# vita-epfl/CrowdNav

Hardware: AMD Instinct MI355X
Metric: env-steps/sec (whole node), 4096 envs x 5 humans, ORCA step (higher is better)
Workload: dtype f32 ORCA solve + f64 env step

## Files before the change

crowdnav_amd/csrc/rollout_fused.h:

```cpp
#pragma once
#include "rollout_kernels.h"

namespace cn {

constexpr int kFusedMaxNC = 5;

template <typename T>
__device__ __forceinline__ T in_vgpr(T x) {
    asm volatile("" : "+v"(x));
    return x;
}

__device__ __forceinline__ void stage_agent(const Params& P, const Smem& s, const Lane& L, const AgentRegs& r,
                                            double human_safety) {
    if (L.lane >= P.nA) return;
    s.kin[L.lane] = make_float4((float)r.px, (float)r.py, (float)r.vx, (float)r.vy);
    s.posd[L.lane] = make_double2(r.px, r.py);
    s.rad[L.lane] = r.rad;
    s.hview[L.lane] = (float)(r.rad + 0.01 + human_safety);
}

__device__ __forceinline__ void preferred_velocity(const AgentRegs& r, float max_speed, bool solve, float4& sol, float4& start) {
    const double gdx = r.gx - r.px, gdy = r.gy - r.py;
    const double speed = norm2(gdx, gdy);
    const float pref_x = (float)(speed > 1.0 ? gdx / speed : gdx);
    const float pref_y = (float)(speed > 1.0 ? gdy / speed : gdy);
    sol = make_float4(pref_x, pref_y, max_speed, solve ? 1.0f : 0.0f);
    float sx, sy;
    lp_start_point(max_speed, pref_x, pref_y, sx, sy);
    start = make_float4(sx, sy, 0.0f, 0.0f);
}

#define CN_FUSED_SYNC() wave_lds_sync()



struct PairRow {
    int my_info, my_slot;
    unsigned long long row_slots;
};
__device__ __forceinline__ PairRow pair_row_of(const Params& P, const Smem& s, int lane) {
    PairRow pr{0, P.nA, 0ull};
    if (lane < P.pairs) {
        pr.my_info = s.pinfo[lane];
        const int c = (pr.my_info >> 16) & 0xff;
        for (int k = 0; k < kFusedMaxNC; ++k) {
            int slot = P.nA;
            if (k < P.NC) {
                const int ik = s.pinfo[lane - c + k];
                slot = ((ik >> 24) & 1) ? ((ik >> 8) & 0xff) : P.nA;
            }
            pr.row_slots |= (unsigned long long)slot << (8 * k);
        }
        pr.my_slot = (int)((pr.row_slots >> (8 * c)) & 0xffull);
    }
    return pr;
}

template <typename Mid>
__device__ __forceinline__ void fused_pair_phase(const Params& P, const Smem& s, const PairRow& pr, float range_sq, Mid&& mid) {
    const int my_info = pr.my_info, my_slot = pr.my_slot;
    const unsigned long long row_slots = pr.row_slots;
    const int q = my_info & 0xff, c = (my_info >> 16) & 0xff;
    const int ol = (my_info >> 8) & 0xff;
    const bool robot_sim = (my_info >> 25) & 1;
    const float4 me = s.kin[q];
    const float4 other = s.kin[my_slot];
    float4 ot[kFusedMaxNC];
#pragma unroll
    for (int k = 0; k < kFusedMaxNC; ++k) ot[k] = s.kin[(int)((row_slots >> (8 * k)) & 0xffull)];
    const float* view = robot_sim ? s.rview : s.hview;
    const float rsum = view[q] + view[ol];
    const float odx = me.x - other.x, ody = me.y - other.y;
    const float mine = odx * odx + ody * ody;
    int rank = 0, within = 0;
    {
        const uint32_t mb = __float_as_uint(mine), rb = __float_as_uint(range_sq);
        uint32_t before = 0u, inside = 0u;
#pragma unroll
        for (int k = 0; k < kFusedMaxNC; ++k) {
            const float dx = me.x - ot[k].x, dy = me.y - ot[k].y;
            const uint32_t vb = __float_as_uint(dx * dx + dy * dy);
            const uint32_t tie = (uint32_t)(k - c) >> 31;
            before = __builtin_amdgcn_alignbit(before, vb - mb - tie, 31);
            inside = __builtin_amdgcn_alignbit(inside, vb - rb, 31);
        }
        within = __popc(inside);
        rank = __popc(before & inside);
    }
    mid();
    if (c == 0) s.count[q] = within < P.orca.max_neighbors ? within : P.orca.max_neighbors;
    if (mine < range_sq && rank < P.orca.max_neighbors)
        s.lines[q * kLineStride + rank] =
            make_half_plane(P.orca, me.x, me.y, me.z, me.w, other.x, other.y, other.z, other.w, rsum);
}

template <int MAXL>
__device__ __forceinline__ void fused_candidates(const Params& P, const Smem& s, int lane) {
    if (lane < P.nA * MAXL) {
        const int q = lane / MAXL, k = lane - q * MAXL;
        const float4 so = s.sol[q];
        const float4* lq = s.lines + q * kLineStride;
        s.cand2[q * kLineStride + k] = lp_line_candidate_pairs5(lq, k, lane, so.z, so.x, so.y);
    }
}

__device__ __forceinline__ void split_barrier() {
    asm volatile("s_waitcnt lgkmcnt(0)\n\ts_barrier" ::: "memory");
}

struct Lp3Item {
    int a, m, i, base;
    bool item;
    float4 li, lj;
    float radius;
};
template <int MAXL>
__device__ __forceinline__ Lp3Item lp3_item_of(const Smem& s, int lane, unsigned long long mask) {
    constexpr int kPairs = MAXL * (MAXL - 1) / 2;
    Lp3Item it;
    const int t = lane / kPairs;
    it.m = lane - t * kPairs;
    it.a = 0;
    unsigned long long rest = mask;
#pragma unroll
    for (int u = 0; u < kWave / kPairs; ++u) {
        const int bit = rest ? __ffsll((long long)rest) - 1 : 0;
        it.a = (u == t) ? bit : it.a;
        rest &= rest - 1ull;
    }
    it.item = lane < (int)__popcll(mask) * kPairs;
    it.i = lp3_program_of(it.m), it.base = it.i * (it.i - 1) / 2;
    const float4* la = s.lines + it.a * kLineStride;
    it.li = la[it.i], it.lj = la[it.m - it.base];
    it.radius = s.sol[it.a].z;
    return it;
}
template <int MAXL>
__device__ __forceinline__ void lp3_head(const Smem& s, const Lp3Item& it) {
    const float4 pr = lp3_project(it.li, it.lj);
    if (it.item) s.proj[it.a * kLineStride + it.m] = pr;
    CN_FUSED_SYNC();
    if (it.item) {
        const float4* pa = s.proj + it.a * kLineStride + it.base;
        s.cand3[it.a * kLineStride + it.m] =
            lp_line_candidate<MAXL - 2>(pa[it.m - it.base], pa, it.m - it.base, it.radius, -it.li.w, it.li.z, true);
    }
}

template <int MAXL>
__device__ __forceinline__ bool split_has_head(unsigned int pred, int u, int n_steps) {
    return pred != 0u && __popc(pred) * (MAXL * (MAXL - 1) / 2) <= kWave && u < n_steps;
}

struct NoOp {
    __device__ __forceinline__ void operator()() const {}
};
template <int MAXL, int BASE_PRIO = 0, typename AfterScan = NoOp>
__device__ __forceinline__ unsigned long long fused_solve(const Params& P, const Smem& s, int lane, bool solve, float& rx,
                                                          float& ry, PhaseClock* clk, unsigned long long have = 0ull,
                                                          AfterScan&& after_scan = NoOp{}) {
    (void)P, (void)clk;
    rx = 0.0f, ry = 0.0f;
    int n = 0, fail = 0;
    if (solve) {
        n = s.count[lane];
        const float4 start = s.res[lane];
        rx = start.x, ry = start.y;
        fail = lp_planar_scan<MAXL>(s.lines + lane * kLineStride, s.cand2 + lane * kLineStride, n, rx, ry);
    }
    CN_TICK(clk, 3);
    const bool need = solve && fail < n;
    const unsigned long long nm = __ballot(need);
#ifdef CN_PHASE_TIMING
    if (clk) clk->acc[9] += __popcll(nm);
#endif
    after_scan();
    if (nm == 0ull) __builtin_amdgcn_s_setprio(BASE_PRIO);
    if (nm != 0ull) {
        __builtin_amdgcn_s_setprio(3);
        constexpr int kPairs = MAXL * (MAXL - 1) / 2;
        const int n_todo = __popcll(nm);
        bool one_pass_done = false;
        if (n_todo * kPairs <= kWave) {
            const Lp3Item it = lp3_item_of<MAXL>(s, lane, nm);
            const bool item = it.item;
            const int a = it.a, i = it.i, m = it.m, base = it.base;
            const float4 li = it.li;
            const float radius = it.radius;
            const bool hit = (nm & ~have) == 0ull;
            if (!hit) {
                lp3_head<MAXL>(s, it);
                CN_FUSED_SYNC();
            }
            if (item && m == base)
                s.cand2[a * kLineStride + i] = lp3_inner_program(s.proj + a * kLineStride, s.cand3 + a * kLineStride, i, li, radius);
            CN_FUSED_SYNC();
            if (need)
                lp3_outer_scan(s.lines + lane * kLineStride, s.cand2 + lane * kLineStride, n, fail, s.sol[lane].z, rx, ry);
            one_pass_done = true;
        } else {
            if (need) s.todo[__popcll(nm & ((1ull << lane) - 1ull))] = lane;
            CN_FUSED_SYNC();
            const int items = n_todo * kPairs;
            for (int p = lane; p < items; p += kWave) {
                const int t = p / kPairs, m = p - t * kPairs;
                const int a = s.todo[t];
                const int i = lp3_program_of(m), j = m - i * (i - 1) / 2;
                const float4* la = s.lines + a * kLineStride;
                s.proj[a * kLineStride + m] = lp3_project(la[i], la[j]);
            }
            CN_FUSED_SYNC();
            for (int p = lane; p < items; p += kWave) {
                const int t = p / kPairs, m = p - t * kPairs;
                const int a = s.todo[t];
                const int i = lp3_program_of(m), base = i * (i - 1) / 2;
                const float4 li = s.lines[a * kLineStride + i];
                const float4* pa = s.proj + a * kLineStride + base;
                s.cand3[a * kLineStride + m] = lp_line_candidate<MAXL - 2>(pa[m - base], pa, m - base, s.sol[a].z, -li.w, li.z, true);
            }
            CN_FUSED_SYNC();
        }
        if (need && !one_pass_done)
            lp3_scan(s.lines + lane * kLineStride, s.proj + lane * kLineStride, s.cand3 + lane * kLineStride, n,
                     fail, s.sol[lane].z, rx, ry);
    }
    return nm;
}

struct StepConsts {
    double dt, limit, limit1, success, collision, ddist, dfactor, hsafety;
};
__device__ __forceinline__ StepConsts step_consts(const Params& P) {
    StepConsts K;
    K.dt = in_vgpr(P.dt), K.limit = in_vgpr(P.time_limit), K.limit1 = in_vgpr(P.time_limit - 1.0);
    K.success = in_vgpr(P.success_reward), K.collision = in_vgpr(P.collision_penalty);
    K.ddist = in_vgpr(P.discomfort_dist), K.dfactor = in_vgpr(P.discomfort_factor);
    K.hsafety = in_vgpr(P.human_safety);
    return K;
}

__device__ __forceinline__ double swept_distance(const AgentRegs& r, bool human, double2 rp, double act_x, double act_y,
                                                 double new_vx, double new_vy, double dt, double robot_rad) {
    const double x1 = r.px - rp.x, y1 = r.py - rp.y;
    const double wx = r.vx - act_x, wy = r.vy - act_y;
    const double x2 = x1 + wx * dt, y2 = y1 + wy * dt;
    const double sx = x2 - x1, sy = y2 - y1;
    double u = ((0.0 - x1) * sx + (0.0 - y1) * sy) / (sx * sx + sy * sy);
    u = (u > 1.0) ? 1.0 : ((u < 0.0) ? 0.0 : u);
    const bool degenerate = (sx == 0.0 && sy == 0.0);
    const double cx = degenerate ? 0.0 - x1 : (x1 + u * sx) - 0.0;
    const double cy = degenerate ? 0.0 - y1 : (y1 + u * sy) - 0.0;
    const double endx = r.px + new_vx * dt, endy = r.py + new_vy * dt;
    const double d = norm2(human ? cx : endx - r.gx, human ? cy : endy - r.gy);
    return human ? d - r.rad - robot_rad : d;
}

struct StepOutcome {
    double reward, dmin;
    int info;
    bool done;
};
__device__ __forceinline__ StepOutcome reduce_env(const Params& P, const Smem& s, int ebase, double gtime, const StepConsts& K) {
    const double goal_dist = s.closest[ebase];
    const double robot_rad = s.rad[ebase];
    double dmin = std::numeric_limits<double>::infinity();
    bool collision = false;
    for (int i = 1; i < P.A; ++i) {
        const double c = s.closest[ebase + i];
        const bool hit = c < 0.0;
        dmin = (!collision & !hit & (c < dmin)) ? c : dmin;
        collision = collision | hit;
    }
    const bool timeout = gtime >= K.limit1;
    const bool reaching = goal_dist < robot_rad;
    const bool danger = dmin < K.ddist;
    double reward = danger ? (dmin - K.ddist) * K.dfactor * K.dt : 0.0;
    int info = danger ? CN_DANGER : CN_NOTHING;
    reward = reaching ? K.success : reward, info = reaching ? CN_REACH_GOAL : info;
    reward = collision ? K.collision : reward, info = collision ? CN_COLLISION : info;
    reward = timeout ? 0.0 : reward, info = timeout ? CN_TIMEOUT : info;
    const bool done = timeout | collision | reaching;
    return StepOutcome{reward, dmin, info, done};
}


#ifdef CN_WAVE_TRACE
static __device__ unsigned long long cn_wave_trace[8192 * 6];
#endif

constexpr int kSplitOrcaPrio = 1;
constexpr int kAssistHead = 1;
#ifndef CN_SPLIT_HEAD_PRIO
#define CN_SPLIT_HEAD_PRIO 2
#endif
#ifndef CN_SPLIT_HEAD_TAIL_PRIO
#define CN_SPLIT_HEAD_TAIL_PRIO 1
#endif

#ifdef CN_SPLIT_PROBE
constexpr bool kSplitProbe = true;
static __device__ unsigned long long cn_split_probe[32];
#define SPLIT_PROBE_DECL()                                                                                   \
    unsigned long long sp_cnt[7] = {}, sp_wait[3] = {}, sp_w1[2] = {}, sp_n1[2] = {}, sp_dt = 0ull; \
    bool sp_prev_head = false
#define SPLIT_PROBE_WAIT(k, barrier)                                   \
    do {                                                               \
        const unsigned long long sp_t0 = __builtin_readcyclecounter(); \
        barrier;                                                       \
        sp_dt = __builtin_readcyclecounter() - sp_t0;                  \
        sp_wait[k] += sp_dt;                                           \
    } while (0)
#define SPLIT_PROBE_AFTER_1(word, head)                               \
    do {                                                               \
        if ((word) != 0u) sp_w1[0] += sp_dt, ++sp_n1[0];               \
        if (sp_prev_head) sp_w1[1] += sp_dt, ++sp_n1[1];               \
        sp_prev_head = (head);                                         \
    } while (0)
#define SPLIT_PROBE_STEP(ended, nm, head, pred)                                  \
    do {                                                                         \
        const bool sp_hit = (head) && (nm) != 0ull && ((nm) & ~(unsigned long long)(pred)) == 0ull; \
        ++sp_cnt[0], sp_cnt[1] += (ended) ? 1 : 0, sp_cnt[2] += (nm) != 0ull ? 1 : 0, sp_cnt[3] += (head) ? 1 : 0; \
        sp_cnt[4] += sp_hit ? 1 : 0, sp_cnt[5] += ((nm) != 0ull && !sp_hit) ? 1 : 0, sp_cnt[6] += ((head) && (nm) == 0ull) ? 1 : 0; \
    } while (0)
#define SPLIT_PROBE_FLUSH(lane, base)                                                        \
    do {                                                                                     \
        if ((lane) == 0) {                                                                   \
            if ((base) == 0)                                                                 \
                for (int k = 0; k < 7; ++k) atomicAdd(&cn_split_probe[k], sp_cnt[k]);        \
            for (int k = 0; k < 3; ++k) atomicAdd(&cn_split_probe[((base) ? 10 : 7) + k], sp_wait[k]); \
            for (int k = 0; k < 2; ++k) {                                                    \
                atomicAdd(&cn_split_probe[((base) ? 17 : 13) + k], sp_w1[k]);                \
                atomicAdd(&cn_split_probe[((base) ? 19 : 15) + k], sp_n1[k]);                \
            }                                                                                \
        }                                                                                    \
    } while (0)
#else
constexpr bool kSplitProbe = false;
#define SPLIT_PROBE_DECL() (void)0
#define SPLIT_PROBE_WAIT(k, barrier) barrier
#define SPLIT_PROBE_AFTER_1(word, head) (void)0
#define SPLIT_PROBE_STEP(ended, nm, head, pred) (void)0
#define SPLIT_PROBE_FLUSH(lane, base) (void)0
#endif

template <int MAXL, int ASSIST>
__device__ __forceinline__ void split_orca_wave(const Params& P, const Smem& s, int n_steps) {
    const int lane = (int)threadIdx.x - kWave;
    float2* const vel = reinterpret_cast<float2*>(s.act);
    const float range_sq = P.orca.neighbor_dist * P.orca.neighbor_dist;
    const double c_dt = in_vgpr(P.dt);
    split_barrier();
    __builtin_amdgcn_s_setprio(kSplitOrcaPrio);
    const PairRow pr = pair_row_of(P, s, lane);
    double px = 0.0, py = 0.0;
    float rx = 0.0f, ry = 0.0f;
    bool solved = false;
    SPLIT_PROBE_DECL();
    for (int u = 0;;) {
        SPLIT_PROBE_WAIT(0, split_barrier());
        const bool ended = __builtin_amdgcn_readfirstlane(s.flag[0]) != 0;
        const unsigned int pred = ((ASSIST & kAssistHead) || kSplitProbe) ? (unsigned int)__builtin_amdgcn_readfirstlane(s.flag[1]) : 0u;
        if (!ended) ++u;
        if (u >= n_steps) {
            split_barrier();
            break;
        }
        const bool head = (ASSIST & kAssistHead) ? split_has_head<MAXL>(pred, u, n_steps) : false;
        SPLIT_PROBE_AFTER_1(pred, head);
        if (lane < P.nA) {
            if (ended) {
                const double2 p = s.posd[lane];
                px = p.x, py = p.y;
            } else if (solved) {
                px = px + (double)rx * c_dt;
                py = py + (double)ry * c_dt;
                s.kin[lane] = make_float4((float)px, (float)py, rx, ry);
            }
        }
        CN_FUSED_SYNC();
        if (lane < P.pairs) fused_pair_phase(P, s, pr, range_sq, [] {});
        SPLIT_PROBE_WAIT(1, split_barrier());
        fused_candidates<MAXL>(P, s, lane);
        CN_FUSED_SYNC();
        solved = lane < P.nA && s.sol[lane < P.nA ? lane : 0].w != 0.0f;
        const unsigned long long nm = fused_solve<MAXL, kSplitOrcaPrio>(P, s, lane, solved, rx, ry, nullptr, head ? pred : 0u, [&] {
            if (head) SPLIT_PROBE_WAIT(2, split_barrier());
        });
        if (lane < P.nA) vel[lane] = make_float2(rx, ry);
        if (((ASSIST & kAssistHead) || kSplitProbe) && lane == 0) s.flag[1] = (int)nm;
        SPLIT_PROBE_STEP(ended, nm, head, pred);
    }
    SPLIT_PROBE_FLUSH(lane, 0);
}

template <bool HEADLINE, bool SPLIT = false, int ASSIST = 0>
__global__ __launch_bounds__((SPLIT ? 2 : 1) * kWave, (SPLIT ? 4 : HEADLINE ? 3 : 1)) void rollout_fused_kernel(
    Params P_in, const StateView* Sd, const int* ring_filled_in, RolloutView R, int n_steps, const double* ext_action) {
    static_assert(HEADLINE || !SPLIT, "the two-wave kernel exists for the headline geometry only");
    static_assert(SPLIT || ASSIST == 0, "the env wave assists an ORCA wave: two-wave kernel only");
#ifdef CN_WAVE_TRACE
    const unsigned long long wt_entry = __builtin_amdgcn_s_memrealtime();
    unsigned long long wt_fallbacks = 0ull, wt_ends = 0ull;
#endif
    constexpr int MAXL = 5;
    Params P = P_in;
    P.async_fill = 0;
    if (HEADLINE) {
        P.A = 6, P.NC = 5, P.E = 2, P.nA = 12, P.pairs = 60, P.threads = 64;
    }
    const Smem s = carve<MAXL>(P);
    if constexpr (SPLIT) {
        if (__builtin_amdgcn_readfirstlane((int)threadIdx.x) >= kWave) {
            split_orca_wave<MAXL, ASSIST>(P, s, n_steps);
            return;
        }
    }
    const Lane L = lane_of(P);
    AgentRegs r = {};
    float robot_max_speed = 0.0f;
    const bool robot = L.valid && L.a == 0;
    const cn_rollout_io* iop = R.io;
    double theta = 0.0;
    EpisodeBook ep = {};
    {
        const StateView S = *Sd;
        const cn_rollout_io io = *iop;
        const size_t gi = L.valid ? L.gi : 0;
        const int env = L.valid ? L.env : 0;
        const double2 p0 = S.pos[gi], v0 = S.vel[gi], g0 = S.goal[gi], q0 = S.rv[gi];
        const bool have = P.robot_orca ? S.rsim_valid[env] != 0 : false;
        const float rr_kept = P.robot_orca ? S.rsim_radius[gi] : 0.0f;
        const float ms_kept = P.robot_orca ? S.rsim_max_speed[env] : 0.0f;
        const double theta0 = S.theta[env];
        EpisodeBook ep0;
        CN_LOAD_EPISODE(P, ep0, S, io, ring_filled_in, env);
        if (L.valid) {
            r.px = p0.x, r.py = p0.y, r.vx = v0.x, r.vy = v0.y, r.gx = g0.x, r.gy = g0.y, r.rad = q0.x, r.vpref = q0.y;
            ep = ep0;
            if (L.a == 0) theta = theta0;
            if (P.robot_orca) {
                const float rr = have ? rr_kept : (float)(r.rad + 0.01 + P.robot_safety);
                if (!have) S.rsim_radius[L.gi] = rr;
                s.rview[L.lane] = rr;
                if (L.a == 0) {
                    robot_max_speed = have ? ms_kept : (float)r.vpref;
                    if (!have) S.rsim_max_speed[L.env] = robot_max_speed;
                }
            }
        }
    }
    build_pairs(P, s);

    if (L.valid && ep.state == kWaitingScenario && scenario_ready(P, *Sd, L.env, ep.ep_count, ep.ring_filled)) {
        load_from_ring(P, *Sd, L, ep.ep_count % P.ring_mod, r);
        ep.state = kRunning;
        ep.gtime = 0.0;
        theta = 1.5707963267948966;
    }
    unsigned int transitions = 0;
    for (int t = threadIdx.x; t < kMaxDiscount; t += P.threads) s.disc[t] = t < R.discount_len ? R.discount[t] : 0.0;
    CN_FUSED_SYNC();
    if (L.lane == 0) s.kin[P.nA] = make_float4(std::numeric_limits<float>::infinity(), std::numeric_limits<float>::infinity(), 0.0f, 0.0f);
    const PairRow pr = pair_row_of(P, s, L.lane);
    const StepConsts K = step_consts(P);
    stage_agent(P, s, L, r, K.hsafety);
    CN_FUSED_SYNC();

#ifdef CN_PHASE_TIMING
    PhaseClock clock = {};
    PhaseClock* clk = &clock;
    clock.last = __builtin_readcyclecounter();
#else
    PhaseClock* clk = nullptr;
    (void)clk;
#endif
    const float range_sq = P.orca.neighbor_dist * P.orca.neighbor_dist;
#ifdef CN_WAVE_TRACE
    const unsigned long long wt_loop = __builtin_amdgcn_s_memrealtime();
#endif
    if constexpr (SPLIT) {
        float2* const vel = reinterpret_cast<float2*>(s.act);
        if (L.lane == 0) s.flag[0] = 1, s.flag[1] = 0;
        split_barrier();
        bool skip = true;
        SPLIT_PROBE_DECL();
        for (int u = 0;;) {
            SPLIT_PROBE_WAIT(0, split_barrier());
            if (!skip) ++u;
            const unsigned int pred = ((ASSIST & kAssistHead) || kSplitProbe) ? (unsigned int)__builtin_amdgcn_readfirstlane(s.flag[1]) : 0u;
            SPLIT_PROBE_AFTER_1(pred, (ASSIST & kAssistHead) != 0 && split_has_head<MAXL>(pred, u, n_steps));
            const bool running = L.valid && ep.state == kRunning;
            const AgentRegs r0 = r;
            double act_x = 0.0, act_y = 0.0, new_vx = 0.0, new_vy = 0.0;
            if (!skip && L.lane < P.nA) {
                const float2 mine = vel[L.lane], robots = vel[L.ebase];
                act_x = (double)robots.x, act_y = (double)robots.y;
                new_vx = (L.a == 0) ? act_x : (double)mine.x;
                new_vy = (L.a == 0) ? act_y : (double)mine.y;
                if (running) {
                    r.px = r.px + new_vx * K.dt;
                    r.py = r.py + new_vy * K.dt;
                    r.vx = new_vx;
                    r.vy = new_vy;
                }
            }
            if (u < n_steps && L.lane < P.nA) {
                float4 sol4, start4;
                preferred_velocity(r, (L.a == 0) ? robot_max_speed : (float)r.vpref, running && (L.a > 0 || P.robot_orca), sol4, start4);
                s.sol[L.lane] = sol4;
                s.res[L.lane] = start4;
            }
            SPLIT_PROBE_WAIT(1, split_barrier());
            if constexpr ((ASSIST & kAssistHead) != 0) {
                if (split_has_head<MAXL>(pred, u, n_steps)) {
                    __builtin_amdgcn_s_setprio(CN_SPLIT_HEAD_PRIO);
                    const Lp3Item it = lp3_item_of<MAXL>(s, L.lane, (unsigned long long)pred);
                    lp3_head<MAXL>(s, it);
                    __builtin_amdgcn_s_setprio(CN_SPLIT_HEAD_TAIL_PRIO);
                    SPLIT_PROBE_WAIT(2, split_barrier());
                }
            }
            bool ended = false;
            if (!skip) {
                const double2 rp = make_double2(__shfl(r0.px, L.ebase), __shfl(r0.py, L.ebase));
                if (L.valid) s.closest[L.lane] = swept_distance(r0, L.a > 0, rp, act_x, act_y, new_vx, new_vy, K.dt, s.rad[L.ebase]);
                CN_FUSED_SYNC();
                bool done = false;
                if (running) {
                    const double disc_t = s.disc[ep.cur_steps < kMaxDiscount ? ep.cur_steps : kMaxDiscount - 1];
                    const StepOutcome o = reduce_env(P, s, L.ebase, ep.gtime, K);
                    done = o.done;
                    ep.gtime += K.dt;
                    ++transitions;
                    CN_BOOK_TRANSITION(ep, ep.cur_steps < kMaxDiscount ? disc_t : 0.0, o.reward, o.info, o.dmin);
                    if (done) {
                        const cn_rollout_io io = *iop;
                        const StateView S = *Sd;
                        AgentRegs next = r;
                        load_from_ring(P, S, L, (ep.ep_count + 1) % P.ring_mod, next);
                        CN_END_EPISODE(P, S, io, L.env, L.a == 0, K.limit, o.info, ep, r = next; theta = 1.5707963267948966);
                    }
                }
                ended = __ballot(done) != 0ull;
            }
            if (ended) stage_agent(P, s, L, r, K.hsafety);
            if (L.lane == 0) s.flag[0] = ended ? 1 : 0;
            skip = ended;
            if constexpr ((ASSIST & kAssistHead) != 0 && CN_SPLIT_HEAD_TAIL_PRIO != 0) __builtin_amdgcn_s_setprio(0);
            if (u >= n_steps) break;
        }
        SPLIT_PROBE_FLUSH(L.lane, 10);
    }
    const int one_wave_steps = SPLIT ? 0 : n_steps;
    for (int step = 0; step < one_wave_steps; ++step) {
        const bool running = L.valid && ep.state == kRunning;
        const bool solve = running && (L.a > 0 || P.robot_orca);

        if (L.lane < P.pairs) {
            float4 sol4, start4;
            fused_pair_phase(P, s, pr, range_sq, [&] {
                preferred_velocity(r, (L.a == 0) ? robot_max_speed : (float)r.vpref, solve, sol4, start4);
            });
            if (L.lane < P.nA) {
                s.sol[L.lane] = sol4;
                s.res[L.lane] = start4;
            }
        }
        CN_FUSED_SYNC();
        CN_TICK(clk, 2);

        fused_candidates<MAXL>(P, s, L.lane);
        CN_FUSED_SYNC();

        float rx, ry;
        const bool fell_back = fused_solve<MAXL>(P, s, L.lane, solve, rx, ry, clk) != 0ull;
        (void)fell_back;
#ifdef CN_WAVE_TRACE
        if (fell_back) ++wt_fallbacks;
#endif
        CN_TICK(clk, 8);

        double act_x, act_y;
        if (P.robot_orca) {
            act_x = (double)__shfl(rx, L.ebase);
            act_y = (double)__shfl(ry, L.ebase);
        } else {
            act_x = L.valid ? ext_action[2 * (size_t)L.env] : 0.0;
            act_y = L.valid ? ext_action[2 * (size_t)L.env + 1] : 0.0;
        }
        const double new_vx = (L.a == 0) ? act_x : (double)rx;
        const double new_vy = (L.a == 0) ? act_y : (double)ry;

        if (L.valid)
            s.closest[L.lane] = swept_distance(r, L.a > 0, s.posd[L.ebase], act_x, act_y, new_vx, new_vy, K.dt, s.rad[L.ebase]);
        CN_FUSED_SYNC();
        CN_TICK(clk, 5);

        if (running) {
            const double disc_t = s.disc[ep.cur_steps < kMaxDiscount ? ep.cur_steps : kMaxDiscount - 1];
            const StepOutcome o = reduce_env(P, s, L.ebase, ep.gtime, K);
            const double reward = o.reward, dmin = o.dmin;
            const int info = o.info;
            const bool done = o.done;
            ep.gtime += K.dt;
            r.px = r.px + new_vx * K.dt;
            r.py = r.py + new_vy * K.dt;
            r.vx = new_vx;
            r.vy = new_vy;
            ++transitions;
            CN_BOOK_TRANSITION(ep, ep.cur_steps < kMaxDiscount ? disc_t : 0.0, reward, info, dmin);
#ifdef CN_WAVE_TRACE
            if (__ballot(done) != 0ull) ++wt_ends;
#endif
            if (done) {
                const cn_rollout_io io = *iop;
                CN_END_EPISODE(P, *Sd, io, L.env, L.a == 0, K.limit, info, ep,
                               load_from_ring(P, *Sd, L, ep.ep_count % P.ring_mod, r); theta = 1.5707963267948966);
            }
        }
        stage_agent(P, s, L, r, K.hsafety);
        CN_FUSED_SYNC();
        CN_TICK(clk, 7);
    }
#ifdef CN_PHASE_TIMING
    if ((threadIdx.x & (kWave - 1)) == 0) {
        unsigned long long total = 0ull;
        for (int k = 0; k < 10; ++k) {
            atomicAdd(&cn_phase_cycles[k], clock.acc[k]);
            if (k != 9) total += clock.acc[k];
        }
        atomicMax(&cn_phase_cycles[14], total);
        atomicMin(&cn_phase_cycles[13], total);
        atomicAdd(&cn_phase_cycles[15], 1ull);
    }
#endif

#ifdef CN_WAVE_TRACE
    const unsigned long long wt_exit = __builtin_amdgcn_s_memrealtime();
#endif
    const StateView S = *Sd;
    if (L.valid) CN_STORE_AGENT(S, L.gi, r);
    const cn_rollout_io io = *iop;
    if (robot) CN_STORE_EPISODE(P, S, io, L.env, ep, theta);
    rollout_epilogue(P, S, io, L, robot, transitions, ep.ep_count, reinterpret_cast<double*>(s.lines));
#ifdef CN_WAVE_TRACE
    if (threadIdx.x == 0 && blockIdx.x < 8192) {
        unsigned long long* w = cn_wave_trace + 6 * blockIdx.x;
        unsigned hw;
        asm volatile("s_getreg_b32 %0, hwreg(HW_REG_HW_ID)" : "=s"(hw));
        w[0] = wt_entry, w[1] = wt_loop, w[2] = wt_exit, w[3] = __builtin_amdgcn_s_memrealtime();
        w[4] = wt_fallbacks | (wt_ends << 32), w[5] = hw;
    }
#endif
}

}
```

Baseline: 1.478 billion.

## Shorten the ORCA wave's step loop with bpermute distances, hoisted loads and mirrored preferred-velocity lanes

The pair phase now fetches neighbour distances from peer lanes with ds_bpermute instead of reloading five kin entries per lane and recomputing them. In the split kernel the ORCA wave does the kin position update at the end of its own step, loads me/other before the ended check, staggers episode-end staging through a separate d2 buffer, and recomputes rsum and solved only when an episode ends. This drops one LDS sync from the common path. The env wave mirrors agent state onto lanes 16+ so the x and y parts of the preferred velocity are computed in parallel and swapped with permlane16_swap. The risk is extra cross-lane state and subtle correctness dependencies, such as stale rsum or solved values, and mirror lanes that need nA <= 16.

```diff
diff --git a/crowdnav_amd/csrc/rollout_fused.h b/crowdnav_amd/csrc/rollout_fused.h
--- a/crowdnav_amd/csrc/rollout_fused.h
+++ b/crowdnav_amd/csrc/rollout_fused.h
@@ -12,9 +12,9 @@
 }
 
 __device__ __forceinline__ void stage_agent(const Params& P, const Smem& s, const Lane& L, const AgentRegs& r,
-                                            double human_safety) {
+                                            double human_safety, float4* kin) {
     if (L.lane >= P.nA) return;
-    s.kin[L.lane] = make_float4((float)r.px, (float)r.py, (float)r.vx, (float)r.vy);
+    kin[L.lane] = make_float4((float)r.px, (float)r.py, (float)r.vx, (float)r.vy);
     s.posd[L.lane] = make_double2(r.px, r.py);
     s.rad[L.lane] = r.rad;
     s.hview[L.lane] = (float)(r.rad + 0.01 + human_safety);
@@ -36,51 +36,45 @@
 
 
 struct PairRow {
-    int my_info, my_slot;
-    unsigned long long row_slots;
+    int my_info, my_slot, xbase;
 };
 __device__ __forceinline__ PairRow pair_row_of(const Params& P, const Smem& s, int lane) {
-    PairRow pr{0, P.nA, 0ull};
+    PairRow pr{0, P.nA, 0};
     if (lane < P.pairs) {
         pr.my_info = s.pinfo[lane];
         const int c = (pr.my_info >> 16) & 0xff;
-        for (int k = 0; k < kFusedMaxNC; ++k) {
-            int slot = P.nA;
-            if (k < P.NC) {
-                const int ik = s.pinfo[lane - c + k];
-                slot = ((ik >> 24) & 1) ? ((ik >> 8) & 0xff) : P.nA;
-            }
-            pr.row_slots |= (unsigned long long)slot << (8 * k);
-        }
-        pr.my_slot = (int)((pr.row_slots >> (8 * c)) & 0xffull);
+        pr.xbase = (lane - c) * 4;
+        pr.my_slot = ((pr.my_info >> 24) & 1) ? ((pr.my_info >> 8) & 0xff) : P.nA;
     }
     return pr;
 }
 
+__device__ __forceinline__ float pair_rsum(const Smem& s, const PairRow& pr) {
+    const int q = pr.my_info & 0xff, ol = (pr.my_info >> 8) & 0xff;
+    const float* view = ((pr.my_info >> 25) & 1) ? s.rview : s.hview;
+    return view[q] + view[ol];
+}
+
 template <typename Mid>
-__device__ __forceinline__ void fused_pair_phase(const Params& P, const Smem& s, const PairRow& pr, float range_sq, Mid&& mid) {
-    const int my_info = pr.my_info, my_slot = pr.my_slot;
-    const unsigned long long row_slots = pr.row_slots;
+__device__ __forceinline__ void fused_pair_body(const Params& P, const Smem& s, const PairRow& pr, float range_sq, float rsum,
+                                                const float4 me, const float4 other, Mid&& mid) {
+    const int my_info = pr.my_info;
     const int q = my_info & 0xff, c = (my_info >> 16) & 0xff;
-    const int ol = (my_info >> 8) & 0xff;
-    const bool robot_sim = (my_info >> 25) & 1;
-    const float4 me = s.kin[q];
-    const float4 other = s.kin[my_slot];
-    float4 ot[kFusedMaxNC];
-#pragma unroll
-    for (int k = 0; k < kFusedMaxNC; ++k) ot[k] = s.kin[(int)((row_slots >> (8 * k)) & 0xffull)];
-    const float* view = robot_sim ? s.rview : s.hview;
-    const float rsum = view[q] + view[ol];
     const float odx = me.x - other.x, ody = me.y - other.y;
     const float mine = odx * odx + ody * ody;
+    uint32_t vbk[kFusedMaxNC];
+#pragma unroll
+    for (int k = 0; k < kFusedMaxNC; ++k) {
+        const uint32_t got = (uint32_t)__builtin_amdgcn_ds_bpermute(pr.xbase + 4 * k, (int)__float_as_uint(mine));
+        vbk[k] = k < P.NC ? got : 0x7f800000u;
+    }
     int rank = 0, within = 0;
     {
         const uint32_t mb = __float_as_uint(mine), rb = __float_as_uint(range_sq);
         uint32_t before = 0u, inside = 0u;
 #pragma unroll
         for (int k = 0; k < kFusedMaxNC; ++k) {
-            const float dx = me.x - ot[k].x, dy = me.y - ot[k].y;
-            const uint32_t vb = __float_as_uint(dx * dx + dy * dy);
+            const uint32_t vb = vbk[k];
             const uint32_t tie = (uint32_t)(k - c) >> 31;
             before = __builtin_amdgcn_alignbit(before, vb - mb - tie, 31);
             inside = __builtin_amdgcn_alignbit(inside, vb - rb, 31);
@@ -93,6 +87,13 @@
     if (mine < range_sq && rank < P.orca.max_neighbors)
         s.lines[q * kLineStride + rank] =
             make_half_plane(P.orca, me.x, me.y, me.z, me.w, other.x, other.y, other.z, other.w, rsum);
+}
+template <typename Mid>
+__device__ __forceinline__ void fused_pair_phase(const Params& P, const Smem& s, const PairRow& pr, float range_sq, float rsum,
+                                                 Mid&& mid) {
+    const float4 me = s.kin[pr.my_info & 0xff];
+    const float4 other = s.kin[pr.my_slot];
+    fused_pair_body(P, s, pr, range_sq, rsum, me, other, mid);
 }
 
 template <int MAXL>
@@ -356,11 +357,15 @@
     double px = 0.0, py = 0.0;
     float rx = 0.0f, ry = 0.0f;
     bool solved = false;
+    float rsum = 0.0f;
+    const int pq = pr.my_info & 0xff;
     SPLIT_PROBE_DECL();
     for (int u = 0;;) {
         SPLIT_PROBE_WAIT(0, split_barrier());
-        const bool ended = __builtin_amdgcn_readfirstlane(s.flag[0]) != 0;
-        const unsigned int pred = ((ASSIST & kAssistHead) || kSplitProbe) ? (unsigned int)__builtin_amdgcn_readfirstlane(s.flag[1]) : 0u;
+        const int2 words = make_int2(s.flag[0], ((ASSIST & kAssistHead) || kSplitProbe) ? s.flag[1] : 0);
+        float4 me = s.kin[pq], other = s.kin[pr.my_slot];
+        const bool ended = __builtin_amdgcn_readfirstlane(words.x) != 0;
+        const unsigned int pred = ((ASSIST & kAssistHead) || kSplitProbe) ? (unsigned int)__builtin_amdgcn_readfirstlane(words.y) : 0u;
         if (!ended) ++u;
         if (u >= n_steps) {
             split_barrier();
@@ -368,27 +373,31 @@
         }
         const bool head = (ASSIST & kAssistHead) ? split_has_head<MAXL>(pred, u, n_steps) : false;
         SPLIT_PROBE_AFTER_1(pred, head);
-        if (lane < P.nA) {
-            if (ended) {
+        if (ended) {
+            if (lane < P.nA) {
                 const double2 p = s.posd[lane];
                 px = p.x, py = p.y;
-            } else if (solved) {
-                px = px + (double)rx * c_dt;
-                py = py + (double)ry * c_dt;
-                s.kin[lane] = make_float4((float)px, (float)py, rx, ry);
-            }
-        }
-        CN_FUSED_SYNC();
-        if (lane < P.pairs) fused_pair_phase(P, s, pr, range_sq, [] {});
+                s.kin[lane] = reinterpret_cast<const float4*>(s.d2)[lane];
+            }
+            CN_FUSED_SYNC();
+            me = s.kin[pq], other = s.kin[pr.my_slot];
+        }
+        if (ended) rsum = pair_rsum(s, pr);
+        if (lane < P.pairs) fused_pair_body(P, s, pr, range_sq, rsum, me, other, [] {});
         SPLIT_PROBE_WAIT(1, split_barrier());
         fused_candidates<MAXL>(P, s, lane);
         CN_FUSED_SYNC();
-        solved = lane < P.nA && s.sol[lane < P.nA ? lane : 0].w != 0.0f;
+        if (ended) solved = lane < P.nA && s.sol[lane < P.nA ? lane : 0].w != 0.0f;
         const unsigned long long nm = fused_solve<MAXL, kSplitOrcaPrio>(P, s, lane, solved, rx, ry, nullptr, head ? pred : 0u, [&] {
             if (head) SPLIT_PROBE_WAIT(2, split_barrier());
         });
         if (lane < P.nA) vel[lane] = make_float2(rx, ry);
         if (((ASSIST & kAssistHead) || kSplitProbe) && lane == 0) s.flag[1] = (int)nm;
+        if (solved) {
+            px = px + (double)rx * c_dt;
+            py = py + (double)ry * c_dt;
+            s.kin[lane] = make_float4((float)px, (float)py, rx, ry);
+        }
         SPLIT_PROBE_STEP(ended, nm, head, pred);
     }
     SPLIT_PROBE_FLUSH(lane, 0);
@@ -464,7 +473,8 @@
     if (L.lane == 0) s.kin[P.nA] = make_float4(std::numeric_limits<float>::infinity(), std::numeric_limits<float>::infinity(), 0.0f, 0.0f);
     const PairRow pr = pair_row_of(P, s, L.lane);
     const StepConsts K = step_consts(P);
-    stage_agent(P, s, L, r, K.hsafety);
+    float4* const kin_stage = SPLIT ? reinterpret_cast<float4*>(s.d2) : s.kin;
+    stage_agent(P, s, L, r, K.hsafety, kin_stage);
     CN_FUSED_SYNC();
 
 #ifdef CN_PHASE_TIMING
@@ -484,6 +494,17 @@
         if (L.lane == 0) s.flag[0] = 1, s.flag[1] = 0;
         split_barrier();
         bool skip = true;
+        const bool mirror = L.lane >= 16 && L.lane < 16 + P.nA;
+        const int m_lane = L.lane & 15;
+        const int m_ebase = __shfl(L.ebase, m_lane);
+        const bool m_robot = __shfl((int)(L.a == 0), m_lane) != 0;
+        bool m_running = false;
+        const auto copy_to_mirror = [&] {
+            const double px = __shfl(r.px, m_lane), py = __shfl(r.py, m_lane), gx = __shfl(r.gx, m_lane), gy = __shfl(r.gy, m_lane);
+            const int run = __shfl((int)(L.valid && ep.state == kRunning), m_lane);
+            if (mirror) r.px = px, r.py = py, r.gx = gx, r.gy = gy, m_running = run != 0;
+        };
+        copy_to_mirror();
         SPLIT_PROBE_DECL();
         for (int u = 0;;) {
             SPLIT_PROBE_WAIT(0, split_barrier());
@@ -493,23 +514,31 @@
             const bool running = L.valid && ep.state == kRunning;
             const AgentRegs r0 = r;
             double act_x = 0.0, act_y = 0.0, new_vx = 0.0, new_vy = 0.0;
-            if (!skip && L.lane < P.nA) {
-                const float2 mine = vel[L.lane], robots = vel[L.ebase];
+            if (!skip && (L.lane < P.nA || mirror)) {
+                const float2 mine = vel[m_lane], robots = vel[m_ebase];
                 act_x = (double)robots.x, act_y = (double)robots.y;
-                new_vx = (L.a == 0) ? act_x : (double)mine.x;
-                new_vy = (L.a == 0) ? act_y : (double)mine.y;
-                if (running) {
+                new_vx = m_robot ? act_x : (double)mine.x;
+                new_vy = m_robot ? act_y : (double)mine.y;
+                if (mirror ? m_running : running) {
                     r.px = r.px + new_vx * K.dt;
                     r.py = r.py + new_vy * K.dt;
                     r.vx = new_vx;
                     r.vy = new_vy;
                 }
             }
-            if (u < n_steps && L.lane < P.nA) {
-                float4 sol4, start4;
-                preferred_velocity(r, (L.a == 0) ? robot_max_speed : (float)r.vpref, running && (L.a > 0 || P.robot_orca), sol4, start4);
-                s.sol[L.lane] = sol4;
-                s.res[L.lane] = start4;
+            if (u < n_steps && (L.lane < P.nA || mirror)) {
+                const double gdx = r.gx - r.px, gdy = r.gy - r.py;
+                const double speed = norm2(gdx, gdy);
+                const double num = mirror ? gdy : gdx;
+                const float pref = (float)(speed > 1.0 ? num / speed : num);
+                const float pref_y = __uint_as_float(__builtin_amdgcn_permlane16_swap(__float_as_uint(pref), __float_as_uint(pref), false, false)[1]);
+                if (L.lane < P.nA) {
+                    const float max_speed = (L.a == 0) ? robot_max_speed : (float)r.vpref;
+                    float sx, sy;
+                    lp_start_point(max_speed, pref, pref_y, sx, sy);
+                    s.sol[L.lane] = make_float4(pref, pref_y, max_speed, (running && (L.a > 0 || P.robot_orca)) ? 1.0f : 0.0f);
+                    s.res[L.lane] = make_float4(sx, sy, 0.0f, 0.0f);
+                }
             }
             SPLIT_PROBE_WAIT(1, split_barrier());
             if constexpr ((ASSIST & kAssistHead) != 0) {
@@ -544,7 +573,8 @@
                 }
                 ended = __ballot(done) != 0ull;
             }
-            if (ended) stage_agent(P, s, L, r, K.hsafety);
+            if (ended) stage_agent(P, s, L, r, K.hsafety, kin_stage);
+            if (ended) copy_to_mirror();
             if (L.lane == 0) s.flag[0] = ended ? 1 : 0;
             skip = ended;
             if constexpr ((ASSIST & kAssistHead) != 0 && CN_SPLIT_HEAD_TAIL_PRIO != 0) __builtin_amdgcn_s_setprio(0);
@@ -559,7 +589,7 @@
 
         if (L.lane < P.pairs) {
             float4 sol4, start4;
-            fused_pair_phase(P, s, pr, range_sq, [&] {
+            fused_pair_phase(P, s, pr, range_sq, pair_rsum(s, pr), [&] {
                 preferred_velocity(r, (L.a == 0) ? robot_max_speed : (float)r.vpref, solve, sol4, start4);
             });
             if (L.lane < P.nA) {
@@ -619,7 +649,7 @@
                                load_from_ring(P, *Sd, L, ep.ep_count % P.ring_mod, r); theta = 1.5707963267948966);
             }
         }
-        stage_agent(P, s, L, r, K.hsafety);
+        stage_agent(P, s, L, r, K.hsafety, kin_stage);
         CN_FUSED_SYNC();
         CN_TICK(clk, 7);
     }
```

Measured after the change: 1.523 billion (median of 6 runs). 1.03x the previous value.
